# barathanaslan/whisper-ipa

Hardware: AMD Instinct MI355X
Metric: audio-seconds/sec transcribed (whisper-small, 30s clips) (higher is better)
Workload: dtype bf16

## Files before the change

include/wipa.h:

```cpp
#ifndef WIPA_H
#define WIPA_H
#include <stddef.h>
#include <stdint.h>
#ifdef __cplusplus
extern "C" {
#endif

typedef void* wipa_stream_t;

enum { WIPA_F32 = 0, WIPA_BF16 = 1, WIPA_FP8_E4M3 = 2  };
enum { WIPA_OK = 0, WIPA_ERR_ARG = -1, WIPA_ERR_HIP = -2, WIPA_ERR_STATE = -3 };

#define WIPA_N_SAMPLES 480000
#define WIPA_N_FRAMES 3000
#define WIPA_N_FFT 400
#define WIPA_HOP 160
#define WIPA_HEAD_DIM 64

int wipa_version(void);
const char* wipa_last_error(void);

int wipa_stream_create(wipa_stream_t* out);
int wipa_stream_create_cu_limited(int n_cus, wipa_stream_t* out);
int wipa_stream_destroy(wipa_stream_t s);
// ... 126 lines not shown
    const float* bqkv;
    const void* wo;
    void* kcache;
    void* vcache;
    const int32_t* pos;
    float* slabs;
    int64_t kv_batch_stride, slab_stride;
    int32_t B, d, H, dtype;
    float eps, qk_scale;
} wipa_self_block_desc;
int wipa_decode_self_block(const wipa_self_block_desc* d, wipa_stream_t s);
typedef struct wipa_cross_block_desc {
    const float* x_in;
    float* x_out;
    const float* slabs;
    const float* bias_o;
    const float* ln_w;
    const float* ln_b;
    const void* wq;
    const float* bq;
    const void* kv;
    void* out;
    int64_t slab_stride;
    int32_t n_slabs, B, d, H, Tk, dtype;
    float eps, qk_scale;
    int32_t cross_splits;
    int32_t n_group;
} wipa_cross_block_desc;
int wipa_decode_cross_block(const wipa_cross_block_desc* d, wipa_stream_t s);

int wipa_cross_absorbed_splits(int want, int Tk);
int wipa_cross_absorbed_resident_groups_for(int B, int d, int Tk, int n_splits, int64_t budget_bytes);
int wipa_cross_absorbed_resident_groups(int B, int d, int Tk, int n_splits);
size_t wipa_cross_absorbed_scratch_bytes(int B, int d, int Tk);
int wipa_cross_absorbed_init(int d);
int wipa_cross_absorbed_attention(const void* q, int64_t q_row_stride, const void* wkT, const void* xa, const void* wv, const float* bv,
                                  void* out, int64_t out_row_stride, void* scratch, size_t scratch_bytes, int B, int H, int d, int Tk,
                                  float k_scale, int n_splits, wipa_stream_t s);
int wipa_cross_absorbed_attention_grouped(const void* q, int64_t q_row_stride, const void* wkT, const void* xa, const void* wv,
                                          const float* bv, void* out, int64_t out_row_stride, void* scratch, size_t scratch_bytes, int B,
                                          int H, int d, int Tk, float k_scale, int n_splits, int n_group, wipa_stream_t s);
int wipa_decode_cross_absorbed_block(const wipa_cross_block_desc* c, const void* wkT, const void* wv, const float* bv, void* scratch,
                                     size_t scratch_bytes, wipa_stream_t s);
int wipa_decode_cross_absorbed_block_out(const wipa_cross_block_desc* c, const void* wkT, const void* wv, const float* bv, const void* wo,
                                         const float* bo, float* slabs_out, int64_t slab_stride, void* scratch, size_t scratch_bytes,
                                         wipa_stream_t s);
int wipa_cross_absorbed_stream(const void* xa, void* scratch, size_t scratch_bytes, int B, int H, int d, int Tk, int n_splits,
                               wipa_stream_t s);

int wipa_greedy_step(const float* logits, int64_t ldl, int B, int V, const float* mask_first,
                     const float* mask_always, int32_t* tokens, int64_t ld_tok, const int32_t* pos_dev, int n_init,
                     int eot, float* sum_logprobs, int32_t* not_done, wipa_stream_t s);
int wipa_add_i32(int32_t* p, int32_t v, wipa_stream_t s);
int wipa_greedy_step_embed(const float* logits, int64_t ldl, int B, int V, const float* mask_first, const float* mask_always,
                           int32_t* tokens, int64_t ld_tok, int32_t* pos_dev, int64_t* posd_dev, int32_t* done_counter, int n_init,
                           int eot, float* sum_logprobs, int32_t* not_done, const void* tok_emb, int emb_dtype,
                           const float* emb_scale, const float* pos_emb, int n_ctx, float* x, const float* ln_w, const float* ln_b,
                           void* y, int y_dtype, int D, float eps, wipa_stream_t s);
#define WIPA_GREEDY_PARTS 2048
int wipa_logits_greedy_supported(int B, int V, int d, int dtype);
size_t wipa_logits_greedy_partials_bytes(int B);
int wipa_logits_greedy(const void* x, int64_t ldx, const void* w, int64_t ldw, float* logits, int64_t ldl, int B, int V, int d,
                       const float* mask_first, const float* mask_always, const int32_t* pos_dev, int n_init, float* partials,
                       size_t partials_bytes, wipa_stream_t s);
int wipa_greedy_step_embed_partials(const float* partials, int n_parts, int B, int32_t* tokens, int64_t ld_tok, int32_t* pos_dev,
                                    int64_t* posd_dev, int32_t* done_counter, int n_init, int eot, float* sum_logprobs,
                                    int32_t* not_done, const void* tok_emb, int emb_dtype, const float* emb_scale, const float* pos_emb,
                                    int n_ctx, float* x, const float* ln_w, const float* ln_b, void* y, int y_dtype, int D, float eps,
                                    wipa_stream_t s);
typedef struct wipa_decode_rules {
    int32_t timestamp_begin;
    int32_t no_timestamps;
    int32_t max_initial_timestamp_index;
} wipa_decode_rules;
// ... 213 lines not shown
```

whisper_ipa_amd/_lib.py:

```python
from __future__ import annotations

import ctypes as C
import os
import threading

_HERE = os.path.dirname(os.path.abspath(__file__))
LIB_PATH = os.path.join(_HERE, "libwipa.so")

WIPA_F32, WIPA_BF16, WIPA_FP8_E4M3 = 0, 1, 2
GREEDY_PARTS = 2048
RESAMPLE_TILE = 512
SCORE_MAX_LEN = 1024
ENC_GLOBAL, ENC_PER_LAYER = 7, 14
DEC_GLOBAL, DEC_PER_LAYER, DEC_FP8_PER_LAYER = 4, 20, 6
GEMM_DISPATCH = ("tile128", "tile256", "tile384", "tile384n", "tile256p", "skinny", "skinny_fp8", "skinny_ln", "kmajor", "split_k",
                 "tile_fp8", "tile_fp8_384")
ENC_FP8_PER_LAYER = 8
DEC_ABSORBED_PER_LAYER = 1

c_void_p, c_int, c_int64, c_size_t, c_float = C.c_void_p, C.c_int, C.c_int64, C.c_size_t, C.c_float


class GemmDesc(C.Structure):
    _fields_ = [
# ... 74 lines not shown
    "wipa_version": (c_int, []),
    "wipa_last_error": (C.c_char_p, []),
    "wipa_stream_create": (c_int, [C.POINTER(c_void_p)]),
    "wipa_stream_create_cu_limited": (c_int, [c_int, C.POINTER(c_void_p)]),
    "wipa_stream_destroy": (c_int, [c_void_p]),
    "wipa_resample_pad": (c_int, [c_void_p, c_size_t, c_void_p, _P(PcmClipDesc), c_int, c_void_p, c_size_t, c_void_p, c_void_p]),
    "wipa_logmel_tables_bytes": (c_size_t, [c_int]),
    "wipa_logmel_init": (c_int, [c_void_p, c_int, c_void_p]),
    "wipa_logmel_workspace_bytes": (c_size_t, [c_int, c_int]),
    "wipa_logmel": (c_int, [c_void_p, c_int, c_int, c_void_p, c_void_p, c_int, c_void_p, c_size_t, c_void_p]),
    "wipa_mel_pad_cast": (c_int, [c_void_p, c_int, c_int, c_void_p, c_int, c_void_p]),
    "wipa_gemm": (c_int, [_P(GemmDesc), c_void_p]),
    "wipa_gemm_dispatch_counts": (c_int, [_P(c_int64), c_int, c_int]),
    "wipa_layernorm": (c_int, [c_void_p, c_int, c_int64, c_void_p, c_int, c_int64, c_void_p, c_void_p, c_int, c_int,
                               c_float, c_void_p]),
    "wipa_layernorm_fp8": (c_int, [c_void_p, c_int64, c_void_p, c_int64, c_void_p, c_void_p, c_void_p, c_int, c_int, c_float, c_void_p]),
    "wipa_rowquant_fp8": (c_int, [c_void_p, c_int, c_int64, c_void_p, c_int64, c_void_p, c_int, c_int, c_void_p]),
    "wipa_add_slabs_layernorm": (c_int, [c_void_p, c_int64, c_void_p, c_int, c_int64, c_void_p, c_int, c_int64, c_void_p,
                                         c_void_p, c_int, c_int, c_float, c_void_p]),
    "wipa_embed_tokens": (c_int, [c_void_p, c_int64, c_int, c_int, c_int, c_void_p, c_void_p, c_int, c_void_p, c_void_p, c_void_p,
                                  c_int, c_void_p]),
    "wipa_attention": (c_int, [_P(AttnDesc), c_void_p]),
    "wipa_flash_attn_enc_f32": (c_int, [c_void_p, c_int64, c_void_p, c_int64, c_void_p, c_int64, c_void_p, c_int64, c_int, c_int,
                                       c_int, c_int, c_void_p]),
    "wipa_flash_attn_enc_bf16": (c_int, [c_void_p, c_int64, c_void_p, c_int64, c_void_p, c_int64, c_int, c_int, c_int,
                                         c_void_p]),
    "wipa_decode_attn": (c_int, [_P(AttnDesc), c_void_p]),
    "wipa_decode_cross_attn": (c_int, [c_void_p, c_void_p, c_void_p, c_int, c_int, c_int, c_int, c_void_p]),
    "wipa_decode_self_block": (c_int, [_P(SelfBlockDesc), c_void_p]),
    "wipa_decode_cross_block": (c_int, [_P(CrossBlockDesc), c_void_p]),
    "wipa_cross_absorbed_splits": (c_int, [c_int, c_int]),
    "wipa_cross_absorbed_resident_groups_for": (c_int, [c_int, c_int, c_int, c_int, c_int64]),
    "wipa_cross_absorbed_resident_groups": (c_int, [c_int, c_int, c_int, c_int]),
    "wipa_cross_absorbed_scratch_bytes": (c_size_t, [c_int, c_int, c_int]),
    "wipa_cross_absorbed_init": (c_int, [c_int]),
    "wipa_cross_absorbed_attention": (c_int, [c_void_p, c_int64, c_void_p, c_void_p, c_void_p, c_void_p, c_void_p, c_int64, c_void_p, c_size_t,
                                              c_int, c_int, c_int, c_int, c_float, c_int, c_void_p]),
    "wipa_cross_absorbed_stream": (c_int, [c_void_p, c_void_p, c_size_t, c_int, c_int, c_int, c_int, c_int, c_void_p]),
    "wipa_decode_cross_absorbed_block": (c_int, [_P(CrossBlockDesc), c_void_p, c_void_p, c_void_p, c_void_p, c_size_t, c_void_p]),
    "wipa_decode_cross_absorbed_block_out": (c_int, [_P(CrossBlockDesc), c_void_p, c_void_p, c_void_p, c_void_p, c_void_p, c_void_p, c_int64,
                                                     c_void_p, c_size_t, c_void_p]),
    "wipa_greedy_step": (c_int, [c_void_p, c_int64, c_int, c_int, c_void_p, c_void_p, c_void_p, c_int64, c_void_p, c_int,
                                 c_int, c_void_p, c_void_p, c_void_p]),
    "wipa_add_i32": (c_int, [c_void_p, C.c_int32, c_void_p]),
    "wipa_greedy_step_embed": (c_int, [c_void_p, c_int64, c_int, c_int, c_void_p, c_void_p, c_void_p, c_int64, c_void_p, c_void_p, c_void_p,
                                       c_int, c_int, c_void_p, c_void_p, c_void_p, c_int, c_void_p, c_void_p, c_int, c_void_p, c_void_p,
                                       c_void_p, c_void_p, c_int, c_int, c_float, c_void_p]),
    "wipa_timestamp_step": (c_int, [c_void_p, c_int64, c_int, c_int, c_void_p, c_void_p, c_void_p, c_int64, c_void_p, c_int, c_int,
                                    _P(DecodeRules), c_void_p, c_void_p, c_void_p]),
    "wipa_timestamp_step_embed": (c_int, [c_void_p, c_int64, c_int, c_int, c_void_p, c_void_p, c_void_p, c_int64, c_void_p, c_void_p, c_void_p,
                                          c_int, c_int, _P(DecodeRules), c_void_p, c_void_p, c_void_p, c_int, c_void_p, c_void_p, c_int,
                                          c_void_p, c_void_p, c_void_p, c_void_p, c_int, c_int, c_float, c_void_p]),
    "wipa_sample_record_bytes": (c_size_t, [c_int]),
    "wipa_sample_record_fill": (c_int, [c_void_p, c_size_t, C.c_uint64, c_int, c_float, c_void_p, c_int]),
    "wipa_sample_step": (c_int, [c_void_p, c_int64, c_int, c_int, c_void_p, c_void_p, c_void_p, c_int64, c_void_p, c_int, c_int,
                                 _P(DecodeRules), c_void_p, c_void_p, c_void_p, c_void_p]),
    "wipa_sample_step_embed": (c_int, [c_void_p, c_int64, c_int, c_int, c_void_p, c_void_p, c_void_p, c_int64, c_void_p, c_void_p, c_void_p,
                                       c_int, c_int, _P(DecodeRules), c_void_p, c_void_p, c_void_p, c_void_p, c_int, c_void_p, c_void_p, c_int,
                                       c_void_p, c_void_p, c_void_p, c_void_p, c_int, c_int, c_float, c_void_p]),
    "wipa_sample_noise": (c_int, [c_void_p, c_int, c_int, c_int, c_void_p, c_void_p]),
    "wipa_logits_greedy_supported": (c_int, [c_int, c_int, c_int, c_int]),
    "wipa_logits_greedy_partials_bytes": (c_size_t, [c_int]),
    "wipa_logits_greedy": (c_int, [c_void_p, c_int64, c_void_p, c_int64, c_void_p, c_int64, c_int, c_int, c_int, c_void_p, c_void_p, c_void_p,
                                   c_int, c_void_p, c_size_t, c_void_p]),
    "wipa_greedy_step_embed_partials": (c_int, [c_void_p, c_int, c_int, c_void_p, c_int64, c_void_p, c_void_p, c_void_p, c_int, c_int, c_void_p,
                                                c_void_p, c_void_p, c_int, c_void_p, c_void_p, c_int, c_void_p, c_void_p, c_void_p, c_void_p,
# ... 130 lines not shown
```

whisper_ipa_amd/csrc/cross_absorbed.hip:

```cpp
#include <cstdlib>
#include <mutex>
#include <type_traits>

#include "attn_stream.h"
#include "wipa_common.h"

int wipa_cross_absorbed_loop_variant() {
    const char* e = getenv("WIPA_ABS_LOOP");
    const int v = e ? atoi(e) : 1;
    return (v >= 0 && v <= 3) ? v : 1;
}

namespace {

constexpr int FT = 32;
constexpr long long XA_RESIDENT_MB_SHARED = 16;
constexpr long long XA_RESIDENT_MB_LONE = -1;
typedef __attribute__((address_space(3))) void* lds_ptr_a;
typedef int v2i32 __attribute__((ext_vector_type(2)));

struct AbsParams {
    const __bf16* qp;
    const __bf16* xa;
    float* part_m;
    float* part_l;
    float* part_o;
    int Tk, n_splits, tiles_per_split, H;
    int resident_groups;
};

template <bool GROUPED>
struct AbsArgs : AbsParams {};
template <>
struct AbsArgs<true> : AbsParams {
    int n_group;
};

constexpr int POLICY_DEFAULT = 0, POLICY_NT = 2;

__device__ __forceinline__ int swz(int row) { return (row & 7) << 1; }

template <int D>
struct AbsCfg {
    static constexpr int NW = 4;
    static constexpr int ROWB = D * 2;
    static constexpr int TILE = FT * ROWB;
    static constexpr int SX = NW * 2 * 64 * 4 * (int)sizeof(float);
    static constexpr int NBUF = (3 * TILE + SX <= 160 * 1024) ? 3 : 2;
    static constexpr int SMEM = NBUF * TILE + SX;
};

template <int D, bool GROUPED = false>
__global__ __launch_bounds__(512, 1) void cross_absorbed_kernel(AbsArgs<GROUPED> p) {
    typedef AbsCfg<D> X;
    constexpr int NW = X::NW, ROWB = X::ROWB, TILE = X::TILE, NBUF = X::NBUF;
    constexpr int NDMA = TILE / 1024 / NW;
    constexpr int KS = D / NW / 32;
    constexpr int CT = D / NW / 16;
    static_assert(D % (32 * NW) == 0 && TILE % (1024 * NW) == 0, "width");
    extern __shared__ __attribute__((aligned(1024))) char smem[];
    float* sx = reinterpret_cast<float*>(smem + NBUF * TILE);
    const int tid = threadIdx.x, lane = tid & 63;
    const int wave = __builtin_amdgcn_readfirstlane(tid >> 6);
    const int l15 = lane & 15, g = lane >> 4;
    const int split = blockIdx.x, b = blockIdx.y;
    const int tile0 = split * p.tiles_per_split;
    const int n_tiles_total = (p.Tk + FT - 1) / FT;
    const int nt = max(0, min(p.tiles_per_split, n_tiles_total - tile0));
    int xclip = b;
    if constexpr (GROUPED) xclip = b / p.n_group;
    const __bf16* xb = p.xa + (int64_t)xclip * p.Tk * D;

    bf16x8 qf[KS];
    {
        const __bf16* qr = p.qp + ((int64_t)b * 16 + l15) * D + wave * (D / NW) + 8 * g;
#pragma unroll
        for (int ks = 0; ks < KS; ++ks) qf[ks] = *reinterpret_cast<const bf16x8*>(qr + 32 * ks);
    }
    const __amdgpu_buffer_rsrc_t rX = __builtin_amdgcn_make_buffer_rsrc((void*)xb, 0, 0x7fffffff, 0x00020000);
    int drow[NDMA], dch[NDMA];
#pragma unroll
    for (int i = 0; i < NDMA; ++i) {
        const int off = 1024 * (NDMA * wave + i) + 16 * lane;
        drow[i] = off / ROWB;
        dch[i] = ((off % ROWB) >> 4) ^ swz(off / ROWB);
    }
    const int res_tiles = p.resident_groups / 2;
    auto stage_as = [&](auto policy, int t, int buf) {
        constexpr int AUX = decltype(policy)::value;
        const int f0 = (tile0 + t) * FT;
#pragma unroll
        for (int i = 0; i < NDMA; ++i) {
            const int voff = min(f0 + drow[i], p.Tk - 1) * ROWB + dch[i] * 16;
            __builtin_amdgcn_raw_ptr_buffer_load_lds(rX, (lds_ptr_a)(smem + buf * TILE + 1024 * (NDMA * wave + i)), 16, voff, 0, 0, AUX);
        }
    };
    auto stage = [&](int t, int buf) {
        if (t < res_tiles) stage_as(std::integral_constant<int, POLICY_DEFAULT>{}, t, buf);
// ... 194 lines not shown
                 : "+v"(X[0]), "+v"(X[1]), "+v"(X[2]), "+v"(X[3]), "+v"(X[4]), "+v"(X[5]), "+v"(X[6]), "+v"(X[7])                   \
                 :                                                                                                                   \
                 : "memory")

__device__ __forceinline__ float max_xor16(float v) {
    const auto r = __builtin_amdgcn_permlane16_swap(__float_as_uint(v), __float_as_uint(v), false, false);
    return fmaxf(__uint_as_float(r[0]), __uint_as_float(r[1]));
}
__device__ __forceinline__ float max_xor32(float v) {
    const auto r = __builtin_amdgcn_permlane32_swap(__float_as_uint(v), __float_as_uint(v), false, false);
    return fmaxf(__uint_as_float(r[0]), __uint_as_float(r[1]));
}
__device__ __forceinline__ float sum_xor16(float v) {
    const auto r = __builtin_amdgcn_permlane16_swap(__float_as_uint(v), __float_as_uint(v), false, false);
    return __uint_as_float(r[0]) + __uint_as_float(r[1]);
}
__device__ __forceinline__ float sum_xor32(float v) {
    const auto r = __builtin_amdgcn_permlane32_swap(__float_as_uint(v), __float_as_uint(v), false, false);
    return __uint_as_float(r[0]) + __uint_as_float(r[1]);
}

template <int D, int NW_, bool PIPE, bool GROUPED = false>
__global__ __launch_bounds__(64 * NW_, 1) void cross_absorbed_v2_kernel(AbsArgs<GROUPED> p) {
    typedef AbsCfg2<D, NW_> X;
    constexpr int NWV = X::NWV, GF = X::GF, ROWB = X::ROWB, SLOT = X::SLOT;
    constexpr int NDMA = SLOT / 1024;
    constexpr int KS = D / 32;
    constexpr int CT = D / 16;
    static_assert(SLOT % 1024 == 0 && NDMA <= 32 && CT % 8 == 0 && KS % 4 == 0 && CT / 8 <= 8 && D % 128 == 0, "width");
    extern __shared__ __attribute__((aligned(1024))) char smem[];
    const int tid = threadIdx.x, lane = tid & 63;
    const int wave = __builtin_amdgcn_readfirstlane(tid >> 6);
    const int l15 = lane & 15, g = lane >> 4;
    const int split = blockIdx.x, b = blockIdx.y;
    const int groups_total = (p.Tk + GF - 1) / GF;
    const int gps = 2 * p.tiles_per_split;
    const int g0 = split * gps;
    const int ng = max(0, min(gps, groups_total - g0));
    const int my_n = ng > wave ? (ng - wave + NWV - 1) / NWV : 0;
    int xclip = b;
    if constexpr (GROUPED) xclip = b / p.n_group;
    const __bf16* xb = p.xa + (int64_t)xclip * p.Tk * D;
    char* my = smem + wave * (2 * SLOT);

    bf16x8 qf[KS];
    {
        const __bf16* qr = p.qp + ((int64_t)b * 16 + l15) * D + 8 * g;
#pragma unroll
        for (int ks = 0; ks < KS; ++ks) qf[ks] = *reinterpret_cast<const bf16x8*>(qr + 32 * ks);
    }
    const __amdgpu_buffer_rsrc_t rX = __builtin_amdgcn_make_buffer_rsrc((void*)xb, 0, 0x7fffffff, 0x00020000);
    constexpr int G1K = (ROWB % 1024 == 0) ? 1024 : ((ROWB % 512 == 0) ? 512 : 256);
    constexpr int PER = ROWB / G1K, QR = 1024 / G1K;
    static_assert(NDMA % PER == 0 && PER <= 3 && (QR == 1 || QR == 2 || QR == 4), "transfer / row period");
    int dma_a[PER], dma_b[PER];
#pragma unroll
    for (int t = 0; t < PER; ++t) {
        const int off = 1024 * t + 16 * lane;
        const int r = off / ROWB, c = (off - r * ROWB) >> 4;
        dma_a[t] = (c ^ (r << 1)) << 4;
        dma_b[t] = r * ROWB;
    }
    int lane_v = lane;
    auto stage_as = [&](auto policy, int i_local, int slot) {
        constexpr int AUX = decltype(policy)::value;
        const int f0 = (g0 + wave + NWV * i_local) * GF;
        if (f0 + GF <= p.Tk) {
// ... 537 lines not shown
    {
        const bf16x8 a0 = *reinterpret_cast<const bf16x8*>(&qh[l15][8 * g]);
        const bf16x8 a1 = *reinterpret_cast<const bf16x8*>(&qh[l15][32 + 8 * g]);
#pragma unroll
        for (int i = 0; i < NTW; ++i) {
            const int nt = wave * NTW + i;
            if (nt < NT) {
                f32x4 acc = {0.f, 0.f, 0.f, 0.f};
                acc = __builtin_amdgcn_mfma_f32_16x16x32_bf16(a0, wkf[i][0], acc, 0, 0, 0);
                acc = __builtin_amdgcn_mfma_f32_16x16x32_bf16(a1, wkf[i][1], acc, 0, 0, 0);
#pragma unroll
                for (int r = 0; r < 4; ++r) {
                    const int bb_ = b0 + 4 * g + r;
                    if (4 * g + r < CG && bb_ < p.B) p.qp[((int64_t)bb_ * 16 + h) * D + 16 * nt + l15] = (__bf16)(acc[r] * p.k_scale);
                }
            }
        }
    }
}

template <int D, bool OUTP, typename... Args>
void launch_merge(int lv, int S, dim3 grid, hipStream_t s, Args... args) {
    constexpr int T = 64 * MergeCfg<D>::NWM;
    const int ns = (lv == 1 || lv == 3) ? S : 4;
    if (ns == 1) hipLaunchKernelGGL((cross_merge_proj_kernel<D, OUTP, 1>), grid, dim3(T), 0, s, args...);
    else if (ns == 2) hipLaunchKernelGGL((cross_merge_proj_kernel<D, OUTP, 2>), grid, dim3(T), 0, s, args...);
    else if (ns == 3) hipLaunchKernelGGL((cross_merge_proj_kernel<D, OUTP, 3>), grid, dim3(T), 0, s, args...);
    else hipLaunchKernelGGL((cross_merge_proj_kernel<D, OUTP, 4>), grid, dim3(T), 0, s, args...);
}

template <int D, bool GROUPED>
int launch_attn_as(int lv, const AbsArgs<GROUPED>& p, int B, hipStream_t s) {
    const char* e = getenv("WIPA_ABS_KERNEL");
    const bool pipe = lv == 1 || lv == 2;
    if ((e && atoi(e) == 1) || (D > 768 && !(e && atoi(e) == 2)))
        hipLaunchKernelGGL((cross_absorbed_kernel<D, GROUPED>), dim3(p.n_splits, B), dim3(64 * AbsCfg<D>::NW), AbsCfg<D>::SMEM, s, p);
    else if constexpr (D > 768) {
        if (pipe) hipLaunchKernelGGL((cross_absorbed_v2_kernel<D, 2, true, GROUPED>), dim3(p.n_splits, B), dim3(128), (AbsCfg2<D, 2>::SMEM), s, p);
        else hipLaunchKernelGGL((cross_absorbed_v2_kernel<D, 2, false, GROUPED>), dim3(p.n_splits, B), dim3(128), (AbsCfg2<D, 2>::SMEM), s, p);
    } else {
        static const int waves = [] { const char* w = getenv("WIPA_ABS_WAVES"); return w ? atoi(w) : 3; }();
        if (waves == 2 && pipe) hipLaunchKernelGGL((cross_absorbed_v2_kernel<D, 2, true, GROUPED>), dim3(p.n_splits, B), dim3(128), (AbsCfg2<D, 2>::SMEM), s, p);
        else if (waves == 2) hipLaunchKernelGGL((cross_absorbed_v2_kernel<D, 2, false, GROUPED>), dim3(p.n_splits, B), dim3(128), (AbsCfg2<D, 2>::SMEM), s, p);
        else if (pipe) hipLaunchKernelGGL((cross_absorbed_v2_kernel<D, 3, true, GROUPED>), dim3(p.n_splits, B), dim3(192), (AbsCfg2<D, 3>::SMEM), s, p);
        else hipLaunchKernelGGL((cross_absorbed_v2_kernel<D, 3, false, GROUPED>), dim3(p.n_splits, B), dim3(192), (AbsCfg2<D, 3>::SMEM), s, p);
    }
    return WIPA_OK;
}
template <int D>
int launch_attn(int lv, const AbsParams& p_in, int B, hipStream_t s, int n_group = 1) {
    if (n_group > 1) {
        AbsArgs<true> p{p_in};
        p.n_group = n_group;
        p.resident_groups = wipa_cross_absorbed_resident_groups(B / n_group, D, p.Tk, p.n_splits);
        return launch_attn_as<D, true>(lv, p, B, s);
    }
    AbsArgs<false> p{p_in};
    p.resident_groups = wipa_cross_absorbed_resident_groups(B, D, p.Tk, p.n_splits);
    return launch_attn_as<D, false>(lv, p, B, s);
}

AbsParams abs_params(void* scratch, int B, int d, int Tk, int S, int H, const void* xa) {
    char* sc = (char*)scratch;
    AbsParams p = {};
    p.qp = (const __bf16*)sc; p.xa = (const __bf16*)xa;
    p.part_m = (float*)(sc + (size_t)B * 16 * d * 2);
    p.part_l = p.part_m + (size_t)B * S * 16;
    p.part_o = p.part_l + (size_t)B * S * 16;
    p.Tk = Tk; p.n_splits = S; p.H = H;
    const int tiles = (Tk + FT - 1) / FT;
    p.tiles_per_split = (tiles + S - 1) / S;
    return p;
}

template <typename F>
int for_width(int d, F f) {
    if (d == 384) return f(std::integral_constant<int, 384>());
    if (d == 512) return f(std::integral_constant<int, 512>());
    if (d == 768) return f(std::integral_constant<int, 768>());
    if (d == 1024) return f(std::integral_constant<int, 1024>());
    return WIPA_ERR_ARG;
}

}

extern "C" int wipa_cross_absorbed_splits(int want, int Tk) {
    const int tiles = (Tk + FT - 1) / FT;
    static const int dflt = [] { const char* e = getenv("WIPA_ABS_SPLITS"); const int v = e ? atoi(e) : 4; return (v >= 1 && v <= 4) ? v : 4; }();
    int s = (want >= 1 && want <= 4) ? want : dflt;
    if (s > tiles / 2) s = tiles / 2;
    return s < 1 ? 1 : s;
}

extern "C" int wipa_cross_absorbed_resident_groups_for(int B, int d, int Tk, int n_splits, int64_t budget_bytes) {
    if (B < 1 || d < 1 || Tk < 1) return 0;
    const int S = wipa_cross_absorbed_splits(n_splits, Tk);
    const int tiles = (Tk + FT - 1) / FT;
    const int gps = 2 * ((tiles + S - 1) / S);
    if (budget_bytes < 0 || budget_bytes >= (int64_t)B * Tk * d * 2) return gps;
    const int64_t g = budget_bytes / ((int64_t)B * S * 16 * d * 2);
    return g < gps ? (int)g : gps;
}

extern "C" int wipa_cross_absorbed_resident_groups(int B, int d, int Tk, int n_splits) {
    static const int64_t env_mb = [] { const char* e = getenv("WIPA_XA_RESIDENT_MB"); return e ? (int64_t)atoll(e) : (int64_t)INT64_MIN; }();
    const int S = wipa_cross_absorbed_splits(n_splits, Tk);
    int64_t mb = env_mb;
    if (mb == INT64_MIN) mb = (S <= 2) ? XA_RESIDENT_MB_SHARED : XA_RESIDENT_MB_LONE;
    return wipa_cross_absorbed_resident_groups_for(B, d, Tk, S, mb < 0 ? -1 : mb * 1000000);
}

extern "C" size_t wipa_cross_absorbed_scratch_bytes(int B, int d, int Tk) {
    (void)Tk;
    return (size_t)B * 16 * d * 2 + (size_t)B * 4 * 16 * (2 + (size_t)d) * 4 + 1024;
}

extern "C" int wipa_cross_absorbed_init(int d) {
    static std::mutex mu;
    static bool done[4] = {false, false, false, false};
    const int wi = d == 384 ? 0 : d == 512 ? 1 : d == 768 ? 2 : d == 1024 ? 3 : -1;
    if (wi < 0) return WIPA_ERR_ARG;
    std::lock_guard<std::mutex> lk(mu);
    if (done[wi]) return WIPA_OK;
    hipError_t e = hipSuccess;
    for_width(d, [&](auto width) {
        constexpr int D = decltype(width)::value;
        e = hipFuncSetAttribute(reinterpret_cast<const void*>(&cross_absorbed_kernel<D>), hipFuncAttributeMaxDynamicSharedMemorySize,
                                AbsCfg<D>::SMEM);
        if constexpr (D <= 768) {
            if (e == hipSuccess)
                e = hipFuncSetAttribute(reinterpret_cast<const void*>(&cross_absorbed_v2_kernel<D, 3, true>),
                                        hipFuncAttributeMaxDynamicSharedMemorySize, AbsCfg2<D, 3>::SMEM);
            if (e == hipSuccess)
                e = hipFuncSetAttribute(reinterpret_cast<const void*>(&cross_absorbed_v2_kernel<D, 3, false>),
                                        hipFuncAttributeMaxDynamicSharedMemorySize, AbsCfg2<D, 3>::SMEM);
        }
        if (e == hipSuccess)
            e = hipFuncSetAttribute(reinterpret_cast<const void*>(&cross_absorbed_v2_kernel<D, 2, true>),
                                    hipFuncAttributeMaxDynamicSharedMemorySize, AbsCfg2<D, 2>::SMEM);
        if (e == hipSuccess)
            e = hipFuncSetAttribute(reinterpret_cast<const void*>(&cross_absorbed_v2_kernel<D, 2, false>),
                                    hipFuncAttributeMaxDynamicSharedMemorySize, AbsCfg2<D, 2>::SMEM);
// ... 149 lines not shown
```

whisper_ipa_amd/csrc/runtime.hip:

```cpp
#include <algorithm>
#include <cstdarg>
#include <cstdlib>
#include <cstring>
#include <strings.h>
#include <map>
#include <mutex>
#include <tuple>
#include <vector>

#include "wipa_common.h"

static thread_local char g_err[512] = "";
void wipa_set_error(const char* fmt, ...) {
    va_list ap;
    va_start(ap, fmt);
    vsnprintf(g_err, sizeof(g_err), fmt, ap);
    va_end(ap);
}
extern "C" const char* wipa_last_error(void) { return g_err; }
extern "C" int wipa_version(void) { return 100; }

extern "C" int wipa_stream_create_cu_limited(int n_cus, wipa_stream_t* out) {
    int dev = 0, total = 0;
    WIPA_CHECK_HIP(hipGetDevice(&dev));
// ... 257 lines not shown
    PROF(PROF_NORM, wipa_layernorm(x, WIPA_F32, d, out, dt, d, (const float*)w[5], (const float*)w[6], M, d, 1e-5f, stream));
    return WIPA_OK;
}

namespace {

constexpr int MAX_SLABS = 4;
inline int group_of(const wipa_model_cfg* c) { return c->dec_n_group > 1 ? c->dec_n_group : 1; }
inline int clips_of(const wipa_model_cfg* c, int B) { return B / group_of(c); }
struct DecScratch {
    size_t x, x2, ln, q, ao, h, slabs, posd, absorbed, greedy_part, total;
};
inline int k_slices_for(int K, int dtype) {
    const int ksteps = K * (int)wipa_dtype_size(dtype) / 64;
    int s = ksteps / 12;
    return s < 1 ? 1 : (s > MAX_SLABS ? MAX_SLABS : s);
}
int decode_mode(const wipa_model_cfg* cfg, int B);
constexpr int MAX_PROMPT = 4;
DecScratch dec_scratch(const wipa_model_cfg* c, int B) {
    const size_t e = wipa_dtype_size(c->dtype), d = c->n_text_state;
    const size_t R = (size_t)B * MAX_PROMPT;
    DecScratch s;
    size_t o = 0;
    s.x = o;    o += align256(R * d * 4);
    s.x2 = o;   o += align256((size_t)B * d * 4);
    s.ln = o;   o += align256(R * d * e);
    s.q = o;    o += align256(R * d * e);
    s.ao = o;   o += align256(R * d * e);
    s.h = o;    o += align256(R * 4 * d * e);
    s.slabs = o; o += align256(std::max((size_t)MAX_SLABS * R, (size_t)c->n_text_head * B) * d * 4);
    s.posd = o; o += 256;
    s.absorbed = o;
    if (c->dec_cross_absorbed) o += align256(wipa_cross_absorbed_scratch_bytes(B, (int)d, c->n_audio_ctx));
    s.greedy_part = o;
    if (wipa_logits_greedy_supported(B, c->n_vocab, (int)d, c->dtype)) o += align256(wipa_logits_greedy_partials_bytes(B));
    s.total = o;
    return s;
}

wipa_dec_layout dec_layout(const wipa_model_cfg* c, int B) {
    const size_t e = wipa_dtype_size(c->dtype);
    const size_t d = c->n_text_state, H = c->n_text_head;
    wipa_dec_layout L;
    size_t o = 0;
    L.ld_tok = c->n_text_ctx + 8;
    L.tokens = o; o += align256((size_t)B * L.ld_tok * 4);
    L.pos = o; o += 256;
    L.not_done = o; o += 256;
    L.sum_logprobs = o; o += align256((size_t)B * 4);
    L.ld_logits = round_up(c->n_vocab, 8);
    L.logits = o; o += align256((size_t)B * L.ld_logits * 4);
    const size_t Bc = clips_of(c, B);
    L.cross_kv = o; o += align256(c->dec_cross_absorbed ? Bc * c->n_audio_ctx * d * e
                                                        : (size_t)c->n_text_layer * Bc * 2 * H * c->n_audio_ctx * 64 * e);
    L.self_kv = o; o += align256((size_t)c->n_text_layer * 3 * B * c->n_text_ctx * d * e);
    L.scratch = o; o += dec_scratch(c, B).total;
    L.total_bytes = o;
    return L;
}

__global__ void advance_pos_kernel(int32_t* pos, int64_t* posd, int d) {
    const int p = *pos + 1;
    *pos = p;
    *posd = (int64_t)p * d;
}

__global__ void fill_tokens_kernel(int32_t* tokens, int64_t ld_tok, int B, int n_init, int i0, int i1, int i2, int i3) {
    const int b = blockIdx.x * blockDim.x + threadIdx.x;
    if (b >= B) return;
    const int first4[4] = {i0, i1, i2, i3};
    for (int t = 0; t < n_init; ++t) tokens[(int64_t)b * ld_tok + t] = first4[t & 3];
}

bool absorbed_block_fused() {
    const char* e = getenv("WIPA_ABS_FUSED_PROLOGUE");
    return !(e && atoi(e) == 0);
}

bool absorbed_merge_out() {
    const char* e = getenv("WIPA_ABS_MERGE_OUT");
    return e && atoi(e) == 1;
}
bool tail_fused() {
    const char* e = getenv("WIPA_DECODE_TAIL");
    return !(e && atoi(e) == 0);
}
struct StepCtx {
    const wipa_decode_rules* rules;
    const void* sample;
    const int32_t* starts;
    int n_init, eot;
    const float *mask_first, *mask_always;
    bool lean;
    bool continuous;
    float* no_speech;
    int no_speech_token;
    const void* sample_rows;
};
bool logits_fused(const wipa_model_cfg* cfg, int B, const StepCtx& c) {
    const char* e = getenv("WIPA_LOGITS_FUSED");
    const bool on = !(e && atoi(e) == 0);
    return on && !c.rules && !c.sample && !c.starts && tail_fused() && cfg->dec_w_dtype == 0 && wipa_logits_greedy_supported(B, cfg->n_vocab, cfg->n_text_state, cfg->dtype);
}
int32_t* done_counter_of(char* st, const wipa_dec_layout& L) { return (int32_t*)(st + L.pos + 64); }

int enqueue_step_head(const wipa_model_cfg* cfg, const void* const* w, char* st, const wipa_dec_layout& L, int B, const StepCtx& ctx,
                      wipa_stream_t stream) {
    const DecScratch S = dec_scratch(cfg, B);
    char* sc = st + L.scratch;
    const void* const* lw0 = w + WIPA_DEC_GLOBAL;
    if (ctx.starts)
        return wipa_embed_layernorm_ragged((const int32_t*)(st + L.tokens), L.ld_tok, B, (const int32_t*)(st + L.pos), ctx.starts, w[0], emb_dtype(cfg),
                                           emb_scale(cfg, w), (const float*)w[1], cfg->n_text_ctx, (float*)(sc + S.x), (const float*)lw0[0],
                                           (const float*)lw0[1], sc + S.ln, cfg->dtype, cfg->n_text_state, 1e-5f, stream);
    return wipa_embed_layernorm((const int32_t*)(st + L.tokens), L.ld_tok, B, (const int32_t*)(st + L.pos), w[0], emb_dtype(cfg), emb_scale(cfg, w),
                                (const float*)w[1], cfg->n_text_ctx, (float*)(sc + S.x), (const float*)lw0[0], (const float*)lw0[1], sc + S.ln,
                                cfg->dtype, cfg->n_text_state, 1e-5f, stream);
// ... 273 lines not shown
    const int P = ctx.n_init, d = cfg->n_text_state;
    float* logits = (float*)(st + L.logits);
    int64_t* posd = (int64_t*)(st + L.scratch + dec_scratch(cfg, B).posd);
    int32_t* tokens = (int32_t*)(st + L.tokens);
    int32_t* pos = (int32_t*)(st + L.pos);
    float* sums = (float*)(st + L.sum_logprobs);
    int32_t* not_done = (int32_t*)(st + L.not_done);
    hipLaunchKernelGGL(set_pos_kernel, dim3(1), dim3(1), 0, (hipStream_t)stream, pos, posd, P - 1, d);
    if (ctx.sample && ctx.starts)
        RT_CALL(wipa_sample_step_ragged(logits, L.ld_logits, B, cfg->n_vocab, ctx.mask_first, ctx.mask_always, tokens, L.ld_tok, pos, P, ctx.eot,
                                        ctx.rules, ctx.sample, ctx.starts, sums, not_done, stream));
    else if (ctx.sample)
        RT_CALL(wipa_sample_step(logits, L.ld_logits, B, cfg->n_vocab, ctx.mask_first, ctx.mask_always, tokens, L.ld_tok, pos, P, ctx.eot, ctx.rules,
                                 ctx.sample, sums, not_done, stream));
    else if (ctx.rules)
        RT_CALL(wipa_timestamp_step(logits, L.ld_logits, B, cfg->n_vocab, ctx.mask_first, ctx.mask_always, tokens, L.ld_tok, pos, P, ctx.eot, ctx.rules,
                                    sums, not_done, stream));
    else
        RT_CALL(wipa_greedy_step(logits, L.ld_logits, B, cfg->n_vocab, ctx.mask_first, ctx.mask_always, tokens, L.ld_tok, pos, P, ctx.eot, sums,
                                 not_done, stream));
    hipLaunchKernelGGL(advance_pos_kernel, dim3(1), dim3(1), 0, (hipStream_t)stream, pos, posd, d);
    WIPA_LAUNCH_CHECK();
    return WIPA_OK;
}

int enqueue_prefill(const wipa_model_cfg* cfg, const void* const* w, char* st, const wipa_dec_layout& L, int B, const StepCtx& ctx,
                    wipa_stream_t stream) {
    const int dt = cfg->dtype;
    const size_t e = wipa_dtype_size(dt);
    const int d = cfg->n_text_state, H = cfg->n_text_head, nctx = cfg->n_text_ctx, Ta = cfg->n_audio_ctx;
    const int P = ctx.n_init, M = B * P;
    const int G = group_of(cfg), Bc = clips_of(cfg, B);
    const DecScratch S = dec_scratch(cfg, B);
    char* sc = st + L.scratch;
    char* ln = sc + S.ln;
    void* q = sc + S.q;
    void* ao = sc + S.ao;
    void* hb = sc + S.h;
    SlabStream r{(float*)(sc + S.x), (float*)(sc + S.slabs), ln, M, d, dt, 1024, 1, stream};
    RT_CALL(wipa_embed_tokens((const int32_t*)(st + L.tokens), L.ld_tok, B, P, 0, nullptr, w[0], emb_dtype(cfg), emb_scale(cfg, w), (const float*)w[1],
                              r.x, d, stream));
    for (int l = 0; l < cfg->n_text_layer; ++l) {
        const void* const* lw = w + WIPA_DEC_GLOBAL + WIPA_DEC_PER_LAYER * l;
        char* skv = st + L.self_kv + (size_t)l * 3 * B * nctx * d * e;
        char* ckv = st + L.cross_kv + (size_t)l * Bc * 2 * H * Ta * 64 * e;
        RT_CALL(r.ln_step(lw[0], lw[1]));
        {
            wipa_gemm_desc g;
            memset(&g, 0, sizeof(g));
            g.stream_weights = 1;
            g.col_scale_n = 2 * d; g.col_scale = QK_SCALE;
            g.rg_in = P; g.rg_valid = P; g.rg_stride = (int64_t)nctx * d;
            g.cg_in = d; g.cg_stride = (int64_t)B * nctx * d;
            RT_CALL(gemm(ln, d, lw[2], d, skv, d, M, 3 * d, d, dt, dt, (const float*)lw[3], 0, nullptr, stream, &g));
        }
        {
            wipa_attn_desc a;
            memset(&a, 0, sizeof(a));
            const size_t slot = (size_t)B * nctx * d * e;
            a.q = skv; a.k = skv + slot; a.v = skv + 2 * slot; a.out = ao;
            a.q_bs = (int64_t)nctx * d; a.q_rs = d; a.q_hs = 64;
            a.k_bs = a.q_bs; a.k_rs = d; a.k_hs = 64;
            a.v_bs = a.q_bs; a.v_rs = d; a.v_hs = 64;
            a.o_bs = (int64_t)P * d; a.o_rs = d; a.o_hs = 64;
            a.B = B; a.H = H; a.Tq = P; a.Tk = P; a.causal = 1; a.dtype = dt;
            RT_CALL(wipa_attention(&a, stream));
        }
        RT_CALL(r.residual_gemm(ao, d, lw[4], lw[5]));
        RT_CALL(r.ln_step(lw[6], lw[7]));
        {
            wipa_gemm_desc g;
            memset(&g, 0, sizeof(g));
            g.stream_weights = 1;
            g.col_scale_n = d; g.col_scale = QK_SCALE;
            RT_CALL(gemm(ln, d, lw[8], d, q, d, M, d, d, dt, dt, (const float*)lw[9], 0, nullptr, stream, &g));
        }
        if (cfg->dec_cross_absorbed) {
            const void* wkT = w[WIPA_DEC_GLOBAL + WIPA_DEC_PER_LAYER * cfg->n_text_layer + WIPA_DEC_ABSORBED_PER_LAYER * l];
            for (int t = 0; t < P; ++t)
                RT_CALL(wipa_cross_absorbed_attention_grouped((const char*)q + (size_t)t * d * e, (int64_t)P * d, wkT, st + L.cross_kv,
                                                              (const char*)lw[10] + (size_t)d * d * e, (const float*)lw[11] + d,
                                                              (char*)ao + (size_t)t * d * e, (int64_t)P * d, sc + S.absorbed,
                                                              S.greedy_part - S.absorbed, B, H, d, Ta, QK_SCALE, cfg->dec_cross_splits, G, stream));
        } else if (G > 1) {
            RT_CALL(wipa_decode_cross_attn_grouped(q, ckv, ao, B, H, Ta, P, G, dt, stream));
        } else {
            RT_CALL(wipa_decode_cross_attn_multi(q, ckv, ao, B, H, Ta, P, dt, stream));
        }
        RT_CALL(r.residual_gemm(ao, d, lw[12], lw[13]));
        RT_CALL(r.ln_step(lw[14], lw[15]));
        {
            wipa_gemm_desc g;
            memset(&g, 0, sizeof(g));
            g.stream_weights = 1;
            RT_CALL(gemm(ln, d, lw[16], d, hb, 4 * d, M, 4 * d, d, dt, dt, (const float*)lw[17], 1, nullptr, stream, &g));
        }
        RT_CALL(r.residual_gemm(hb, 4 * d, lw[18], lw[19]));
    }
    RT_CALL(r.ln_step(w[2], w[3]));
    RT_CALL(gemm(ln + (size_t)(P - 1) * d * e, (int64_t)P * d, w[0], d, st + L.logits, L.ld_logits, B, cfg->n_vocab, d, dt, WIPA_F32, nullptr, 0,
                 nullptr, stream));
    return enqueue_first_token(cfg, st, L, B, ctx, stream);
}

bool counters_attached() {
    const char* e = getenv("ROCPROF_COUNTER_COLLECTION");
    return e && *e && strcmp(e, "0") != 0 && strcasecmp(e, "false") != 0;
}
bool graphs_allowed() {
    const char* g = getenv("WIPA_DECODE_GRAPH");
    if (g && (strcmp(g, "0") == 0 || strcasecmp(g, "off") == 0)) return false;
    if (g && strcasecmp(g, "force") == 0) return true;
// ... 34 lines not shown
    WIPA_REQUIRE(B % G == 0, "%s: B=%d rows are no multiple of cfg.dec_n_group=%d (rows = clips x candidates)", who, B, G);
    if (G == 1) return WIPA_OK;
    WIPA_REQUIRE(tail_fused() && !use_fused_step(cfg, B),
                 "%s: sampling lives in the fused step tail; WIPA_DECODE_TAIL=0 / WIPA_DECODE_FUSED=1 cannot serve it", who);
    return WIPA_OK;
}
int starts_servable(const char* who, const wipa_model_cfg* cfg, int B, int n_init, const int32_t* starts_dev) {
    if (!starts_dev) return WIPA_OK;
    WIPA_REQUIRE(tail_fused() && !use_fused_step(cfg, B),
                 "%s: starts_dev (ragged prompts) needs the unfused step with the fused tail; WIPA_DECODE_TAIL=0 / WIPA_DECODE_FUSED=1 cannot serve it", who);
    WIPA_REQUIRE(cfg->dec_w_dtype == 0, "%s: starts_dev (ragged prompts) is not served on fp8 decoder tables (cfg.dec_w_dtype)", who);
    WIPA_REQUIRE(n_init >= 1 && n_init <= cfg->n_text_ctx, "%s: prompt width P=%d outside 1..n_text_ctx=%d", who, n_init, cfg->n_text_ctx);
    return WIPA_OK;
}
int rules_servable(const char* who, const wipa_model_cfg* cfg, int B, int eot, const wipa_decode_rules* r) {
    if (!r) return WIPA_OK;
    WIPA_REQUIRE(tail_fused() && !use_fused_step(cfg, B),
                 "%s: the timestamp rules live in the fused step tail; WIPA_DECODE_TAIL=0 / WIPA_DECODE_FUSED=1 cannot serve them", who);
    WIPA_REQUIRE(r->timestamp_begin > 0 && r->timestamp_begin < cfg->n_vocab && eot < r->timestamp_begin && r->no_timestamps >= 0 &&
                     r->no_timestamps < r->timestamp_begin && cfg->n_vocab <= 65536,
                 "%s: need eot < timestamp_begin < n_vocab <= 65536 and no_timestamps below timestamp_begin (eot=%d timestamp_begin=%d "
                 "no_timestamps=%d n_vocab=%d)", who, eot, r->timestamp_begin, r->no_timestamps, cfg->n_vocab);
    return WIPA_OK;
}
std::mutex g_graph_mu;
std::map<GraphKey, hipGraphExec_t> g_graphs;

bool lean_steps(const wipa_model_cfg* cfg, int B, const StepCtx& c) { return !use_fused_step(cfg, B) && logits_fused(cfg, B, c); }
int step_variant(const wipa_model_cfg* cfg, int B, const StepCtx& c) {
    return cfg->dtype * 2 + t_f32_split + 4 * decode_mode(cfg, B) + 16 * cfg->dec_w_dtype +
           64 * cfg->dec_cross_absorbed * (absorbed_block_fused() ? 2 : 1) + 256 * (int)tail_fused() + 512 * (int)absorbed_merge_out() +
           1024 * cfg->dec_cross_splits + 8192 * (int)lean_steps(cfg, B, c) +
           16384 * (cfg->dec_cross_absorbed ? wipa_cross_absorbed_loop_variant() : 0) + 65536 * (group_of(cfg) > 1 ? group_of(cfg) : 0) +
           (1 << 28) * (int)c.continuous + (1 << 29) * (int)(c.continuous && c.rules) + (1 << 30) * (int)(c.continuous && c.sample_rows);
}
GraphKey graph_key(const wipa_model_cfg* cfg, const void* const* w, const void* state, int B, const StepCtx& c, int variant, int kind,
                   const void* workspace) {
    return GraphKey(state, (const void*)w, (const void*)c.mask_first, (const void*)c.mask_always, B, c.n_init, c.eot, variant,
                    cfg->weights_generation, kind, c.rules ? c.rules->timestamp_begin : 0, c.rules ? c.rules->no_timestamps : 0,
                    c.rules ? c.rules->max_initial_timestamp_index : 0, c.sample ? c.sample : c.sample_rows, (const void*)c.starts, workspace,
                    (const void*)c.no_speech, c.no_speech ? c.no_speech_token : 0);
}
template <typename Enqueue>
int cached_graph(const GraphKey& key, hipStream_t s, Enqueue&& enqueue, hipGraphExec_t* out) {
    hipGraphExec_t exec = nullptr;
    {
        std::lock_guard<std::mutex> lk(g_graph_mu);
        auto it = g_graphs.find(key);
        if (it != g_graphs.end()) exec = it->second;
    }
    if (!exec) {
        hipGraph_t graph = nullptr;
        WIPA_CHECK_HIP(hipStreamBeginCapture(s, hipStreamCaptureModeRelaxed));
        const int rc = enqueue();
        const hipError_t ee = hipStreamEndCapture(s, &graph);
        if (rc != WIPA_OK) {
            if (graph) hipGraphDestroy(graph);
            return rc;
        }
        WIPA_CHECK_HIP(ee);
        WIPA_CHECK_HIP(hipGraphInstantiate(&exec, graph, nullptr, nullptr, 0));
        WIPA_CHECK_HIP(hipGraphDestroy(graph));
        std::lock_guard<std::mutex> lk(g_graph_mu);
        g_graphs[key] = exec;
    }
    *out = exec;
// ... 829 lines not shown
```

Before: 27440.

## Batch prompt-token cross-attention into one grouped absorbed launch with clip-major grid

Replaces the per-prompt-position loop of absorbed cross-attention launches in the prompt/prefill pass with a single grouped launch covering all M=B*P rows, treating P*G rows as sharing one clip's audio context. The grouped kernel moves to a 1-D grid whose block ids are interleaved so that the 8 consecutive blocks are different splits/clips while rows of the same clip-split are adjacent, aiming for L2 reuse of the shared cross KV. Scratch is sized by R rows instead of B, and the graph variant key gains a bit for the new path. This cuts P separate kernel launches at the cost of a different scheduling order and relying on scratch being large enough.

```diff
diff --git a/include/wipa.h b/include/wipa.h
--- a/include/wipa.h
+++ b/include/wipa.h
@@ -182,6 +182,7 @@
 int wipa_cross_absorbed_splits(int want, int Tk);
 int wipa_cross_absorbed_resident_groups_for(int B, int d, int Tk, int n_splits, int64_t budget_bytes);
 int wipa_cross_absorbed_resident_groups(int B, int d, int Tk, int n_splits);
+int wipa_cross_absorbed_resident_groups_rows(int C, int R, int d, int Tk, int n_splits);
 size_t wipa_cross_absorbed_scratch_bytes(int B, int d, int Tk);
 int wipa_cross_absorbed_init(int d);
 int wipa_cross_absorbed_attention(const void* q, int64_t q_row_stride, const void* wkT, const void* xa, const void* wv, const float* bv,
@@ -190,6 +191,8 @@
 int wipa_cross_absorbed_attention_grouped(const void* q, int64_t q_row_stride, const void* wkT, const void* xa, const void* wv,
                                           const float* bv, void* out, int64_t out_row_stride, void* scratch, size_t scratch_bytes, int B,
                                           int H, int d, int Tk, float k_scale, int n_splits, int n_group, wipa_stream_t s);
+int wipa_cross_absorbed_group_grid(int S, int C, int R);
+int wipa_cross_absorbed_group_block(int id, int S, int C, int R, int* split, int* row);
 int wipa_decode_cross_absorbed_block(const wipa_cross_block_desc* c, const void* wkT, const void* wv, const float* bv, void* scratch,
                                      size_t scratch_bytes, wipa_stream_t s);
 int wipa_decode_cross_absorbed_block_out(const wipa_cross_block_desc* c, const void* wkT, const void* wv, const float* bv, const void* wo,
diff --git a/whisper_ipa_amd/_lib.py b/whisper_ipa_amd/_lib.py
--- a/whisper_ipa_amd/_lib.py
+++ b/whisper_ipa_amd/_lib.py
@@ -130,6 +130,9 @@
     "wipa_cross_absorbed_splits": (c_int, [c_int, c_int]),
     "wipa_cross_absorbed_resident_groups_for": (c_int, [c_int, c_int, c_int, c_int, c_int64]),
     "wipa_cross_absorbed_resident_groups": (c_int, [c_int, c_int, c_int, c_int]),
+    "wipa_cross_absorbed_resident_groups_rows": (c_int, [c_int, c_int, c_int, c_int, c_int]),
+    "wipa_cross_absorbed_group_grid": (c_int, [c_int, c_int, c_int]),
+    "wipa_cross_absorbed_group_block": (c_int, [c_int, c_int, c_int, c_int, _P(C.c_int32), _P(C.c_int32)]),
     "wipa_cross_absorbed_scratch_bytes": (c_size_t, [c_int, c_int, c_int]),
     "wipa_cross_absorbed_init": (c_int, [c_int]),
     "wipa_cross_absorbed_attention": (c_int, [c_void_p, c_int64, c_void_p, c_void_p, c_void_p, c_void_p, c_void_p, c_int64, c_void_p, c_size_t,
diff --git a/whisper_ipa_amd/csrc/cross_absorbed.hip b/whisper_ipa_amd/csrc/cross_absorbed.hip
--- a/whisper_ipa_amd/csrc/cross_absorbed.hip
+++ b/whisper_ipa_amd/csrc/cross_absorbed.hip
@@ -34,7 +34,20 @@
 template <>
 struct AbsArgs<true> : AbsParams {
     int n_group;
+    int n_clips;
 };
+
+__host__ __device__ inline int abs_group_grid(int S, int C, int R) { return 8 * R * ((S * C + 7) / 8); }
+__host__ __device__ inline bool abs_group_block(int id, int S, int C, int R, int* split, int* row) {
+    const int res = id & 7, k = id >> 3;
+    const int t = k % R, blk = k / R;
+    const int u = res + 8 * blk;
+    if (id < 0 || u >= S * C) return false;
+    const int clip = u / S;
+    *split = u % S;
+    *row = clip * R + t;
+    return true;
+}
 
 constexpr int POLICY_DEFAULT = 0, POLICY_NT = 2;
 
@@ -63,7 +76,10 @@
     const int tid = threadIdx.x, lane = tid & 63;
     const int wave = __builtin_amdgcn_readfirstlane(tid >> 6);
     const int l15 = lane & 15, g = lane >> 4;
-    const int split = blockIdx.x, b = blockIdx.y;
+    int split = blockIdx.x, b = blockIdx.y;
+    if constexpr (GROUPED) {
+        if (!abs_group_block((int)blockIdx.x, p.n_splits, p.n_clips, p.n_group, &split, &b)) return;
+    }
     const int tile0 = split * p.tiles_per_split;
     const int n_tiles_total = (p.Tk + FT - 1) / FT;
     const int nt = max(0, min(p.tiles_per_split, n_tiles_total - tile0));
@@ -324,7 +340,10 @@
     const int tid = threadIdx.x, lane = tid & 63;
     const int wave = __builtin_amdgcn_readfirstlane(tid >> 6);
     const int l15 = lane & 15, g = lane >> 4;
-    const int split = blockIdx.x, b = blockIdx.y;
+    int split = blockIdx.x, b = blockIdx.y;
+    if constexpr (GROUPED) {
+        if (!abs_group_block((int)blockIdx.x, p.n_splits, p.n_clips, p.n_group, &split, &b)) return;
+    }
     const int groups_total = (p.Tk + GF - 1) / GF;
     const int gps = 2 * p.tiles_per_split;
     const int g0 = split * gps;
@@ -928,18 +947,20 @@
 template <int D, bool GROUPED>
 int launch_attn_as(int lv, const AbsArgs<GROUPED>& p, int B, hipStream_t s) {
     const char* e = getenv("WIPA_ABS_KERNEL");
+    dim3 grid(p.n_splits, B);
+    if constexpr (GROUPED) grid = dim3(abs_group_grid(p.n_splits, p.n_clips, p.n_group));
     const bool pipe = lv == 1 || lv == 2;
     if ((e && atoi(e) == 1) || (D > 768 && !(e && atoi(e) == 2)))
-        hipLaunchKernelGGL((cross_absorbed_kernel<D, GROUPED>), dim3(p.n_splits, B), dim3(64 * AbsCfg<D>::NW), AbsCfg<D>::SMEM, s, p);
+        hipLaunchKernelGGL((cross_absorbed_kernel<D, GROUPED>), grid, dim3(64 * AbsCfg<D>::NW), AbsCfg<D>::SMEM, s, p);
     else if constexpr (D > 768) {
-        if (pipe) hipLaunchKernelGGL((cross_absorbed_v2_kernel<D, 2, true, GROUPED>), dim3(p.n_splits, B), dim3(128), (AbsCfg2<D, 2>::SMEM), s, p);
-        else hipLaunchKernelGGL((cross_absorbed_v2_kernel<D, 2, false, GROUPED>), dim3(p.n_splits, B), dim3(128), (AbsCfg2<D, 2>::SMEM), s, p);
+        if (pipe) hipLaunchKernelGGL((cross_absorbed_v2_kernel<D, 2, true, GROUPED>), grid, dim3(128), (AbsCfg2<D, 2>::SMEM), s, p);
+        else hipLaunchKernelGGL((cross_absorbed_v2_kernel<D, 2, false, GROUPED>), grid, dim3(128), (AbsCfg2<D, 2>::SMEM), s, p);
     } else {
         static const int waves = [] { const char* w = getenv("WIPA_ABS_WAVES"); return w ? atoi(w) : 3; }();
-        if (waves == 2 && pipe) hipLaunchKernelGGL((cross_absorbed_v2_kernel<D, 2, true, GROUPED>), dim3(p.n_splits, B), dim3(128), (AbsCfg2<D, 2>::SMEM), s, p);
-        else if (waves == 2) hipLaunchKernelGGL((cross_absorbed_v2_kernel<D, 2, false, GROUPED>), dim3(p.n_splits, B), dim3(128), (AbsCfg2<D, 2>::SMEM), s, p);
-        else if (pipe) hipLaunchKernelGGL((cross_absorbed_v2_kernel<D, 3, true, GROUPED>), dim3(p.n_splits, B), dim3(192), (AbsCfg2<D, 3>::SMEM), s, p);
-        else hipLaunchKernelGGL((cross_absorbed_v2_kernel<D, 3, false, GROUPED>), dim3(p.n_splits, B), dim3(192), (AbsCfg2<D, 3>::SMEM), s, p);
+        if (waves == 2 && pipe) hipLaunchKernelGGL((cross_absorbed_v2_kernel<D, 2, true, GROUPED>), grid, dim3(128), (AbsCfg2<D, 2>::SMEM), s, p);
+        else if (waves == 2) hipLaunchKernelGGL((cross_absorbed_v2_kernel<D, 2, false, GROUPED>), grid, dim3(128), (AbsCfg2<D, 2>::SMEM), s, p);
+        else if (pipe) hipLaunchKernelGGL((cross_absorbed_v2_kernel<D, 3, true, GROUPED>), grid, dim3(192), (AbsCfg2<D, 3>::SMEM), s, p);
+        else hipLaunchKernelGGL((cross_absorbed_v2_kernel<D, 3, false, GROUPED>), grid, dim3(192), (AbsCfg2<D, 3>::SMEM), s, p);
     }
     return WIPA_OK;
 }
@@ -948,7 +969,8 @@
     if (n_group > 1) {
         AbsArgs<true> p{p_in};
         p.n_group = n_group;
-        p.resident_groups = wipa_cross_absorbed_resident_groups(B / n_group, D, p.Tk, p.n_splits);
+        p.n_clips = B / n_group;
+        p.resident_groups = wipa_cross_absorbed_resident_groups_rows(B / n_group, n_group, D, p.Tk, p.n_splits);
         return launch_attn_as<D, true>(lv, p, B, s);
     }
     AbsArgs<false> p{p_in};
@@ -1004,6 +1026,22 @@
     int64_t mb = env_mb;
     if (mb == INT64_MIN) mb = (S <= 2) ? XA_RESIDENT_MB_SHARED : XA_RESIDENT_MB_LONE;
     return wipa_cross_absorbed_resident_groups_for(B, d, Tk, S, mb < 0 ? -1 : mb * 1000000);
+}
+
+extern "C" int wipa_cross_absorbed_resident_groups_rows(int C, int R, int d, int Tk, int n_splits) {
+    static const int64_t env_mb = [] { const char* e = getenv("WIPA_XA_RESIDENT_ROWS_MB"); return e ? (int64_t)atoll(e) : (int64_t)INT64_MIN; }();
+    if (R < 1) return 0;
+    if (env_mb == INT64_MIN) return wipa_cross_absorbed_resident_groups(C, d, Tk, n_splits);
+    return wipa_cross_absorbed_resident_groups_for(C, d, Tk, wipa_cross_absorbed_splits(n_splits, Tk), env_mb < 0 ? -1 : env_mb * 1000000);
+}
+
+extern "C" int wipa_cross_absorbed_group_grid(int S, int C, int R) {
+    if (S < 1 || C < 1 || R < 1) return 0;
+    return abs_group_grid(S, C, R);
+}
+extern "C" int wipa_cross_absorbed_group_block(int id, int S, int C, int R, int* split, int* row) {
+    if (S < 1 || C < 1 || R < 1 || !split || !row || id < 0 || id >= abs_group_grid(S, C, R)) return 0;
+    return abs_group_block(id, S, C, R, split, row) ? 1 : 0;
 }
 
 extern "C" size_t wipa_cross_absorbed_scratch_bytes(int B, int d, int Tk) {
diff --git a/whisper_ipa_amd/csrc/runtime.hip b/whisper_ipa_amd/csrc/runtime.hip
--- a/whisper_ipa_amd/csrc/runtime.hip
+++ b/whisper_ipa_amd/csrc/runtime.hip
@@ -313,7 +313,7 @@
     s.slabs = o; o += align256(std::max((size_t)MAX_SLABS * R, (size_t)c->n_text_head * B) * d * 4);
     s.posd = o; o += 256;
     s.absorbed = o;
-    if (c->dec_cross_absorbed) o += align256(wipa_cross_absorbed_scratch_bytes(B, (int)d, c->n_audio_ctx));
+    if (c->dec_cross_absorbed) o += align256(wipa_cross_absorbed_scratch_bytes((int)R, (int)d, c->n_audio_ctx));
     s.greedy_part = o;
     if (wipa_logits_greedy_supported(B, c->n_vocab, (int)d, c->dtype)) o += align256(wipa_logits_greedy_partials_bytes(B));
     s.total = o;
@@ -365,6 +365,10 @@
 }
 bool tail_fused() {
     const char* e = getenv("WIPA_DECODE_TAIL");
+    return !(e && atoi(e) == 0);
+}
+bool prompt_chain() {
+    const char* e = getenv("WIPA_PROMPT_CHAIN");
     return !(e && atoi(e) == 0);
 }
 struct StepCtx {
@@ -704,6 +708,7 @@
     const int P = ctx.n_init, M = B * P;
     const int G = group_of(cfg), Bc = clips_of(cfg, B);
     const DecScratch S = dec_scratch(cfg, B);
+    const bool chain = prompt_chain() && M <= 65535;
     char* sc = st + L.scratch;
     char* ln = sc + S.ln;
     void* q = sc + S.q;
@@ -749,7 +754,11 @@
         }
         if (cfg->dec_cross_absorbed) {
             const void* wkT = w[WIPA_DEC_GLOBAL + WIPA_DEC_PER_LAYER * cfg->n_text_layer + WIPA_DEC_ABSORBED_PER_LAYER * l];
-            for (int t = 0; t < P; ++t)
+            if (chain)
+                RT_CALL(wipa_cross_absorbed_attention_grouped(q, d, wkT, st + L.cross_kv, (const char*)lw[10] + (size_t)d * d * e,
+                                                              (const float*)lw[11] + d, ao, d, sc + S.absorbed, S.greedy_part - S.absorbed, M, H,
+                                                              d, Ta, QK_SCALE, cfg->dec_cross_splits, P * G, stream));
+            else for (int t = 0; t < P; ++t)
                 RT_CALL(wipa_cross_absorbed_attention_grouped((const char*)q + (size_t)t * d * e, (int64_t)P * d, wkT, st + L.cross_kv,
                                                               (const char*)lw[10] + (size_t)d * d * e, (const float*)lw[11] + d,
                                                               (char*)ao + (size_t)t * d * e, (int64_t)P * d, sc + S.absorbed,
@@ -850,6 +859,7 @@
            64 * cfg->dec_cross_absorbed * (absorbed_block_fused() ? 2 : 1) + 256 * (int)tail_fused() + 512 * (int)absorbed_merge_out() +
            1024 * cfg->dec_cross_splits + 8192 * (int)lean_steps(cfg, B, c) +
            16384 * (cfg->dec_cross_absorbed ? wipa_cross_absorbed_loop_variant() : 0) + 65536 * (group_of(cfg) > 1 ? group_of(cfg) : 0) +
+           (1 << 27) * (int)(cfg->dec_cross_absorbed && prompt_chain()) +
            (1 << 28) * (int)c.continuous + (1 << 29) * (int)(c.continuous && c.rules) + (1 << 30) * (int)(c.continuous && c.sample_rows);
 }
 GraphKey graph_key(const wipa_model_cfg* cfg, const void* const* w, const void* state, int B, const StepCtx& c, int variant, int kind,
```

After: 27570 (median of 6 runs). About the same (+0.5%).
